# google-research/multinerf

Hardware: NVIDIA H100
Metric: train-step rays/sec @16384 rays x (64+64+32) samples (higher is better)
Workload: dtype bf16

## Files before the change

include/mnrf.h:

```cpp
#ifndef MNRF_H_
#define MNRF_H_

#include <stddef.h>
#include <stdint.h>

#ifdef __cplusplus
extern "C" {
#endif

typedef uint16_t mnrf_bf16;
typedef void* mnrf_stream;

#define MNRF_ABI_VERSION 2

int mnrf_abi_version(void);
const char* mnrf_last_error(void);
int mnrf_device_ok(void);
int mnrf_num_sms(void);

typedef struct {
  int32_t num_rays, num_prev, num_samples;
  int32_t use_dilation;
  float dilation, domain_lo, domain_hi;
  float anneal, resample_padding;
// ... 74 lines not shown
enum { MNRF_CHAIN_FWD = 0, MNRF_CHAIN_BWD = 1 };

typedef struct {
  const mnrf_bf16* w;
  int64_t ldw;
  const float* bias;
  uint32_t* maskbits;
  int64_t ldmaskbits;
  float* colsum;
  mnrf_bf16* out;
  int64_t ldo;
  int32_t n_stream, stream_col0, stream_kb0;
  int32_t n_res, res_kb0;
  int32_t reserved;
} mnrf_chain_layer;

typedef struct {
  int32_t mode, num_layers;
  int32_t width;
  int32_t stream_cols;
  int64_t m;
  const mnrf_bf16* stream;
  int64_t ldstream;
  const float* head_w;
  const float* head_b;
  float* head_out;
  int32_t head_n;
  int32_t reserved;
  mnrf_chain_layer layer[MNRF_CHAIN_MAX_LAYERS];
} mnrf_chain_desc;

int mnrf_mlp_chain(const mnrf_chain_desc* d, mnrf_stream stream);
int mnrf_mlp_chain_max_layers(void);

int mnrf_head_fwd(int64_t m, int32_t k, int32_t n_out, const mnrf_bf16* x, int64_t ldx,
                  const mnrf_bf16* w, const float* b, float* raw, mnrf_stream stream);
int mnrf_head_bwd(int64_t m, int32_t k, int32_t n_out, const mnrf_bf16* x, int64_t ldx,
                  const mnrf_bf16* w, const float* draw, mnrf_bf16* dx, int64_t lddx,
                  int32_t act, const mnrf_bf16* z, int64_t ldz, float* dw, float* dw2, int32_t dw_split,
                  float* db, float* dxsum, int32_t dx_cols, mnrf_bf16* dx2, int64_t lddx2, mnrf_stream stream);

enum { MNRF_HEAD_NONE = 0, MNRF_HEAD_FWD_SUB = 1, MNRF_HEAD_FWD_WARP = 2, MNRF_HEAD_BWD_SUB = 3,
       MNRF_HEAD_BWD_WARP = 4 };
typedef struct {
  int32_t fwd_kernel;
  int32_t fwd_lpr;
  int32_t fwd_grid;
  int32_t bwd_kernel;
  int32_t bwd_n_out;
  int32_t bwd_lpr;
  int32_t bwd_chunks;
  int32_t bwd_smooth;
  int32_t bwd_grid;
  int32_t reserved;
  int64_t fwd_rows_per_pass;
  int64_t bwd_rows_per_block;
} mnrf_head_instance;
int mnrf_head_plan(int64_t m, int32_t k, int32_t n_out, const mnrf_bf16* x, const mnrf_bf16* w, int32_t act,
                   const mnrf_bf16* z, const mnrf_bf16* dx, mnrf_head_instance* plan);

int mnrf_colsum(int64_t m, int32_t n, const mnrf_bf16* x, int64_t ldx, float* out,
                mnrf_stream stream);

enum { MNRF_RGB_SIGMOID = 0, MNRF_RGB_SAFE_EXP = 1 };

typedef struct {
// ... 218 lines not shown
```

multinerf_b200/csrc/chain.cu:

```cuda
#include <stdlib.h>
#include <string.h>

#include <algorithm>

#include "tc_common.cuh"

namespace mnrf {

constexpr int CH_W = 256;
constexpr int CH_ROWS = 128;
constexpr int CH_KBLK = CH_ROWS * 128;
constexpr int CH_WBLK = CH_W * 128;
constexpr int CH_RING = 4;
constexpr int CH_SEG = CH_W / 64;
constexpr int CH_SBLK = 64 * 128;
constexpr int CH_SRING = 3;
constexpr int CH_ACT = 4 * CH_KBLK;
constexpr int CH_THREADS = 384;
constexpr int CH_MAX_LAYERS = MNRF_CHAIN_MAX_LAYERS;
constexpr int CH_AUX = CH_MAX_LAYERS * CH_W * 4;
constexpr int CH_SMEM = CH_ACT + CH_RING * CH_WBLK + CH_SRING * CH_SBLK + CH_AUX + 256  + 1024 ;
static_assert(CH_SMEM <= 232448, "shared memory budget");
static_assert(CH_SEG >= 1 && CH_SEG <= CH_RING, "a segment must fit in the weight ring");

struct alignas(64) ChainMaps {
  CUtensorMap stream;
  CUtensorMap w[CH_MAX_LAYERS];
  CUtensorMap out[CH_MAX_LAYERS];
};

struct ChainLayer {
  int n_stream, stream_col0, stream_kb0;
  int n_res, res_kb0;
  int store;
  const float* bias;
  uint32_t* maskbits;
  int64_t ldmaskbits;
  float* colsum;
};

struct ChainParams {
  int num_layers;
  int64_t m;
  int64_t num_units;
  ChainLayer layer[CH_MAX_LAYERS];
  const float* head_w;
  const float* head_b;
  float* head_out;
};

__device__ __forceinline__ uint32_t pack_bf16_relu(float lo, float hi) {
  uint32_t r;
  asm("cvt.rn.relu.bf16x2.f32 %0, %1, %2;" : "=r"(r) : "f"(hi), "f"(lo));
  return r;
}

__device__ __forceinline__ float2 ld_shared_const_f2(uint32_t addr) {
  float2 v;
  asm("ld.shared.v2.f32 {%0, %1}, [%2];" : "=f"(v.x), "=f"(v.y) : "r"(addr));
  return v;
}

enum { CK_TURN, CK_FULL, CK_MMA, CK_EPI_SYNC, CK_EPI_LOOP, CK_EPI_TAIL, CK_N };
#ifdef MNRF_CHAIN_CLOCKS
__device__ unsigned long long g_chain_clk[CK_N];
#define CH_CLK(k) do { const long long t_ = clock64(); clk[k] += t_ - clk_t; clk_t = t_; } while (0)
#else
#define CH_CLK(k) do { } while (0)
#endif

template <int MODE, int NH>
__global__ void __launch_bounds__(CH_THREADS, 1)
mlp_chain_kernel(const __grid_constant__ ChainMaps maps, const ChainParams p) {
  extern __shared__ uint8_t smem_dyn[];
  uint8_t* smem = reinterpret_cast<uint8_t*>((reinterpret_cast<uintptr_t>(smem_dyn) + 1023) & ~uintptr_t(1023));
  uint8_t* act = smem;
  uint8_t* wring = act + CH_ACT;
  uint8_t* sring = wring + CH_RING * CH_WBLK;
  float* aux = reinterpret_cast<float*>(sring + CH_SRING * CH_SBLK);
  uint64_t* wfull = reinterpret_cast<uint64_t*>(aux + CH_MAX_LAYERS * CH_W);
  uint64_t* wempty = wfull + CH_RING;
  uint64_t* sfull = wempty + CH_RING;
  uint64_t* sempty = sfull + CH_SRING;
  uint64_t* turn = sempty + CH_SRING;

  const int warp = threadIdx.x >> 5;
  const int lane = threadIdx.x & 31;
  const int wg = threadIdx.x >> 7;

  if (threadIdx.x == 0) {
    bool any_stream = false;
    for (int j = 0; j < p.num_layers; ++j) {
      prefetch_tmap(&maps.w[j]);
      if (p.layer[j].store) prefetch_tmap(&maps.out[j]);
      any_stream |= p.layer[j].n_stream > 0;
    }
    if (any_stream) prefetch_tmap(&maps.stream);
    for (int i = 0; i < CH_RING; ++i) { mbar_init(&wfull[i], 1); mbar_init(&wempty[i], 8); }
    for (int i = 0; i < CH_SRING; ++i) { mbar_init(&sfull[i], 1); mbar_init(&sempty[i], 4); }
    for (int i = 0; i < 2; ++i) mbar_init(&turn[i], 4);
    fence_barrier_init();
  }
  if (MODE == 1)
    for (int i = threadIdx.x; i < CH_MAX_LAYERS * CH_W; i += CH_THREADS) aux[i] = 0.f;
  __syncthreads();
  pdl_launch_dependents();
  pdl_wait();
  if (MODE == 0) {
    for (int i = threadIdx.x; i < p.num_layers * CH_W; i += CH_THREADS) aux[i] = __ldg(p.layer[i / CH_W].bias + i % CH_W);
    __syncthreads();
  }

  if (wg == 0) {
    setmaxnreg_dec<40>();
    if (threadIdx.x == 0) {
      uint32_t wslot = 0, wphase = 0, sslot = 0, sphase = 0;
      for (int64_t unit = blockIdx.x; unit < p.num_units; unit += gridDim.x) {
        const int row0 = (int)(unit * CH_ROWS);
        for (int j = 0; j < p.num_layers; ++j) {
          const ChainLayer& L = p.layer[j];
          const int nk = L.n_res + L.n_stream;
          for (int s0 = 0; s0 < nk; s0 += CH_SEG) {
            const int s1 = min(s0 + CH_SEG, nk);
            for (int c = 0; c < 2; ++c)
              for (int s = s0; s < s1; ++s) {
                const bool streamed = s >= L.n_res;
                const int si = s - L.n_res;
                if (c == 0) {
                  mbar_wait(&wempty[wslot], wphase ^ 1, 1);
                  mbar_expect_tx(&wfull[wslot], CH_WBLK);
                  tma_load_2d(wring + wslot * CH_WBLK, &maps.w[j], &wfull[wslot],
                              (streamed ? L.stream_kb0 + si : L.res_kb0 + s) * 64, 0);
                  if (++wslot == CH_RING) { wslot = 0; wphase ^= 1; }
                }
                if (streamed) {
                  mbar_wait(&sempty[sslot], sphase ^ 1, 2);
                  mbar_expect_tx(&sfull[sslot], CH_SBLK);
                  tma_load_2d(sring + sslot * CH_SBLK, &maps.stream, &sfull[sslot], L.stream_col0 + si * 64, row0 + 64 * c);
                  if (++sslot == CH_SRING) { sslot = 0; sphase ^= 1; }
                }
              }
          }
          if (j == 0 && L.n_stream > 0 && unit + gridDim.x < p.num_units)
            for (int si = 0; si < L.n_stream; ++si)
              for (int c = 0; c < 2; ++c)
                tma_prefetch_2d(&maps.stream, L.stream_col0 + si * 64, (int)((unit + gridDim.x) * CH_ROWS) + 64 * c);
        }
      }
    }
  } else {
    setmaxnreg_inc<232>();
    const int c = wg - 1;
    const int w = warp & 3;
    const int r_in = 64 * c + 16 * w + (lane >> 2);
    const int q = lane & 3;
    const int cq = 2 * q;
    const uint32_t wring_s = smem_u32(wring), sring_s = smem_u32(sring), act_s = smem_u32(act);
    const uint32_t aux_s = smem_u32(aux);
    const bool lead = (threadIdx.x & 127) == 0;
    uint32_t wslot = 0, wphase = 0;
    uint32_t spos = 0;
    uint32_t seg = 0;
#ifdef MNRF_CHAIN_CLOCKS
    long long clk[CK_N] = {};
    long long clk_t = clock64();
#endif
    float acc[CH_W / 2];
    for (int64_t unit = blockIdx.x; unit < p.num_units; unit += gridDim.x) {
      int64_t rows[2];
      bool row_ok[2];
#pragma unroll
      for (int h = 0; h < 2; ++h) {
        rows[h] = unit * CH_ROWS + r_in + 8 * h;
        row_ok[h] = rows[h] < p.m;
      }
      for (int j = 0; j < p.num_layers; ++j) {
        const ChainLayer& L = p.layer[j];
        const bool last = (j == p.num_layers - 1);
        const bool do_head = (MODE == 0) && last && p.head_w != nullptr;
        uint32_t mw[2][2] = {{0u, 0u}, {0u, 0u}};
        if (MODE == 1 && L.maskbits) {
#pragma unroll
          for (int h = 0; h < 2; ++h)
#pragma unroll
            for (int e = 0; e < 2; ++e)
              if (row_ok[h]) mw[h][e] = __ldg(L.maskbits + rows[h] * L.ldmaskbits + 2 * q + e);
        }
        const int nk = L.n_res + L.n_stream;
        fence_acc(acc);
        for (int s0 = 0; s0 < nk; s0 += CH_SEG, ++seg) {
          const int s1 = min(s0 + CH_SEG, nk);
          const int ns = s1 - max(s0, L.n_res);
          uint32_t sp = spos + (c && ns > 0 ? ns : 0);
          if (ns > 0) spos += 2 * ns;
          if (c == 1) mbar_wait(&turn[1], seg & 1, 7);
          else if (seg > 0) mbar_wait(&turn[0], (seg - 1) & 1, 7);
          CH_CLK(CK_TURN);
          int prev_w = -1, prev_s = -1;
          for (int s = s0; s < s1; ++s) {
            const bool streamed = s >= L.n_res;
            mbar_wait(&wfull[wslot], wphase, 3);
            uint32_t a0 = act_s + s * CH_KBLK + c * (64 * 128);
            int cur_s = -1;
            if (streamed) {
              cur_s = (int)(sp % CH_SRING);
              mbar_wait(&sfull[cur_s], (sp / CH_SRING) & 1, 4);
              a0 = sring_s + cur_s * CH_SBLK;
              ++sp;
            }
            CH_CLK(CK_FULL);
            const uint32_t b0 = wring_s + wslot * CH_WBLK;
            wgmma_fence();
#pragma unroll
            for (int k = 0; k < 64 / WGMMA_K; ++k)
              Wgmma<CH_W, 0, 0>::mma(acc, make_smem_desc(a0 + k * (WGMMA_K * 2), 0, 1024),
                                     make_smem_desc(b0 + k * (WGMMA_K * 2), 0, 1024), (s > 0 || k > 0) ? 1u : 0u);
            wgmma_commit();
            wgmma_wait<1>();
            if (lane == 0) {
              if (prev_w >= 0) mbar_arrive(&wempty[prev_w]);
              if (prev_s >= 0) mbar_arrive(&sempty[prev_s]);
            }
            prev_w = (int)wslot;
            prev_s = cur_s;
            if (++wslot == CH_RING) { wslot = 0; wphase ^= 1; }
          }
          __syncwarp();
          if (lane == 0) mbar_arrive(&turn[c ^ 1]);
          wgmma_wait<0>();
          if (lane == 0) {
            mbar_arrive(&wempty[prev_w]);
            if (prev_s >= 0) mbar_arrive(&sempty[prev_s]);
          }
          CH_CLK(CK_MMA);
        }
        fence_acc(acc);

        if (lead) tma_store_wait_read<0>();
        named_bar_sync(1 + c, 128);
        CH_CLK(CK_EPI_SYNC);
        uint32_t bits[2] = {0u, 0u};
        float hdot[NH][2];
#pragma unroll
        for (int o = 0; o < NH; ++o) hdot[o][0] = hdot[o][1] = 0.f;
#pragma unroll
        for (int i = 0; i < CH_W / 8; ++i) {
          const int col = 8 * i + cq;
          float v[2][2];
#pragma unroll
          for (int h = 0; h < 2; ++h) { v[h][0] = acc[4 * i + 2 * h]; v[h][1] = acc[4 * i + 2 * h + 1]; }
          uint32_t o[2];
          if (MODE == 0) {
            const float2 b = ld_shared_const_f2(aux_s + (j * CH_W + col) * 4);
#pragma unroll
            for (int h = 0; h < 2; ++h) {
              v[h][0] += b.x;
              v[h][1] += b.y;
              bits[h] |= ((v[h][0] > 0.f ? 1u : 0u) | (v[h][1] > 0.f ? 2u : 0u)) << (col & 31);
              o[h] = pack_bf16_relu(v[h][0], v[h][1]);
            }
            if (do_head) {
#pragma unroll
              for (int oo = 0; oo < NH; ++oo) {
                const float2 hw = __ldg(reinterpret_cast<const float2*>(p.head_w + oo * CH_W + col));
#pragma unroll
                for (int h = 0; h < 2; ++h) hdot[oo][h] += bf16_lo(o[h]) * hw.x + bf16_hi(o[h]) * hw.y;
              }
            }
          } else {
            if (L.maskbits && (i & 3) == 0) {
#pragma unroll
              for (int h = 0; h < 2; ++h)
                bits[h] = __shfl_sync(0xffffffffu, mw[h][(i >> 2) & 1], (lane & ~3) | (i >> 3));
            }
#pragma unroll
            for (int h = 0; h < 2; ++h) {
              if (L.maskbits) {
                if (!((bits[h] >> (col & 31)) & 1u)) v[h][0] = 0.f;
                if (!((bits[h] >> ((col + 1) & 31)) & 1u)) v[h][1] = 0.f;
              }
              o[h] = pack_bf16(v[h][0], v[h][1]);
            }
            if (L.colsum) {
              float s0 = v[0][0] + v[1][0], s1 = v[0][1] + v[1][1];
#pragma unroll
              for (int sh = 4; sh < 32; sh <<= 1) {
                s0 += __shfl_xor_sync(0xffffffffu, s0, sh);
                s1 += __shfl_xor_sync(0xffffffffu, s1, sh);
              }
              if (lane < 4) { atomicAdd(aux + j * CH_W + col, s0); atomicAdd(aux + j * CH_W + col + 1, s1); }
            }
          }
#pragma unroll
          for (int h = 0; h < 2; ++h) {
            const int r = r_in + 8 * h;
            st_shared_u32(act_s + (col >> 6) * CH_KBLK + r * 128 + ((((col & 63) >> 3) ^ (r & 7)) << 4) + (cq << 1), o[h]);
          }
          if (MODE == 0 && (i & 3) == 3) {
#pragma unroll
            for (int h = 0; h < 2; ++h) {
              bits[h] |= __shfl_xor_sync(0xffffffffu, bits[h], 1);
              bits[h] |= __shfl_xor_sync(0xffffffffu, bits[h], 2);
              if (q == (i >> 3)) mw[h][(i >> 2) & 1] = bits[h];
              bits[h] = 0u;
            }
          }
        }
        CH_CLK(CK_EPI_LOOP);
        fence_proxy_async();
        named_bar_sync(1 + c, 128);
        CH_CLK(CK_EPI_SYNC);
        if (lead && L.store) {
#pragma unroll
          for (int kb = 0; kb < 4; ++kb)
            tma_store_2d(&maps.out[j], act + kb * CH_KBLK + c * (64 * 128), kb * 64, (int)(unit * CH_ROWS) + 64 * c);
          tma_store_commit();
        }
        if (MODE == 0 && L.maskbits) {
          const bool wide = (((uintptr_t)L.maskbits | (uintptr_t)(L.ldmaskbits * 4)) & 7) == 0;
#pragma unroll
          for (int h = 0; h < 2; ++h) {
            if (!row_ok[h]) continue;
            uint32_t* dst = L.maskbits + rows[h] * L.ldmaskbits + 2 * q;
            if (wide) *reinterpret_cast<uint2*>(dst) = make_uint2(mw[h][0], mw[h][1]);
            else { dst[0] = mw[h][0]; dst[1] = mw[h][1]; }
          }
        }
        if (do_head) {
#pragma unroll
          for (int oo = 0; oo < NH; ++oo)
#pragma unroll
            for (int h = 0; h < 2; ++h) {
              hdot[oo][h] += __shfl_xor_sync(0xffffffffu, hdot[oo][h], 1);
              hdot[oo][h] += __shfl_xor_sync(0xffffffffu, hdot[oo][h], 2);
              if (q == 0 && row_ok[h])
                p.head_out[rows[h] * NH + oo] = hdot[oo][h] + (p.head_b ? __ldg(p.head_b + oo) : 0.f);
            }
        }
        CH_CLK(CK_EPI_TAIL);
      }
    }
    if (lead) tma_store_wait_all();
#ifdef MNRF_CHAIN_CLOCKS
    if (blockIdx.x == 0 && threadIdx.x == 256)
      for (int k = 0; k < CK_N; ++k) atomicAdd(&g_chain_clk[k], (unsigned long long)clk[k]);
#endif
    if (MODE == 1) {
      named_bar_sync(3, 256);
      for (int jj = 0; jj < p.num_layers; ++jj) {
        if (!p.layer[jj].colsum) continue;
        for (int i = threadIdx.x - 128; i < CH_W; i += 256) atomicAdd(p.layer[jj].colsum + i, aux[jj * CH_W + i]);
      }
    }
  }
}

}

extern "C" int mnrf_mlp_chain_max_layers(void) { return mnrf::CH_MAX_LAYERS; }

#ifdef MNRF_CHAIN_CLOCKS
extern "C" int mnrf_chain_clocks(unsigned long long* out) {
  unsigned long long zero[mnrf::CK_N] = {};
  if (cudaDeviceSynchronize() != cudaSuccess) return 1;
  if (cudaMemcpyFromSymbol(out, mnrf::g_chain_clk, sizeof(zero)) != cudaSuccess) return 1;
  return cudaMemcpyToSymbol(mnrf::g_chain_clk, zero, sizeof(zero)) != cudaSuccess;
}
#endif

extern "C" int mnrf_mlp_chain(const mnrf_chain_desc* d, mnrf_stream stream_) {
  using namespace mnrf;
  cudaStream_t stream = (cudaStream_t)stream_;
  MNRF_CHECK(d, "mnrf_mlp_chain: null descriptor");
  MNRF_CHECK(d->m >= 0 && (d->m + CH_ROWS - 1) / CH_ROWS * CH_ROWS <= INT32_MAX,
             "mnrf_mlp_chain: m must be in [0, %d], got %lld", INT32_MAX / CH_ROWS * CH_ROWS, (long long)d->m);
  if (d->m == 0) return 0;
  MNRF_CHECK(d->mode == MNRF_CHAIN_FWD || d->mode == MNRF_CHAIN_BWD, "mnrf_mlp_chain: bad mode %d", d->mode);
  MNRF_CHECK(d->num_layers >= 1 && d->num_layers <= CH_MAX_LAYERS, "mnrf_mlp_chain: 1..%d layers, got %d",
             CH_MAX_LAYERS, d->num_layers);
  MNRF_CHECK(d->width == CH_W, "mnrf_mlp_chain: layer width must be %d, got %d", CH_W, d->width);
  const int sms = mnrf_num_sms();
  ChainMaps maps;
  memset(&maps, 0, sizeof(maps));
  ChainParams p{};
  p.num_layers = d->num_layers;
  p.m = d->m;
  p.num_units = (d->m + CH_ROWS - 1) / CH_ROWS;
  bool any_stream = false;
  for (int j = 0; j < d->num_layers; ++j) {
    const mnrf_chain_layer& s = d->layer[j];
    ChainLayer& L = p.layer[j];
    MNRF_CHECK(s.n_res == 0 || s.n_res == CH_W / 64, "mnrf_mlp_chain: layer %d: n_res must be 0 or %d", j, CH_W / 64);
    MNRF_CHECK(s.n_stream >= 0 && (s.n_stream > 0 || s.n_res > 0), "mnrf_mlp_chain: layer %d has no operand", j);
    MNRF_CHECK(s.stream_col0 >= 0 && s.stream_kb0 >= 0 && s.res_kb0 >= 0,
               "mnrf_mlp_chain: layer %d: negative column or k-block offset", j);
    MNRF_CHECK(j > 0 || s.n_res == 0, "mnrf_mlp_chain: the first layer has no resident operand");
    MNRF_CHECK(s.w && ((uintptr_t)s.w % 16) == 0 && s.ldw % 8 == 0, "mnrf_mlp_chain: layer %d: weights must be 16-byte aligned", j);
    const int kblocks = std::max(s.n_stream > 0 ? s.stream_kb0 + s.n_stream : 0, s.n_res > 0 ? s.res_kb0 + s.n_res : 0);
    MNRF_CHECK(s.ldw >= (int64_t)kblocks * 64, "mnrf_mlp_chain: layer %d: weight pitch %lld < K %d", j, (long long)s.ldw, kblocks * 64);
    L.n_stream = s.n_stream; L.stream_col0 = s.stream_col0; L.stream_kb0 = s.stream_kb0;
    L.n_res = s.n_res; L.res_kb0 = s.res_kb0;
    L.store = s.out ? 1 : 0;
    L.bias = s.bias; L.maskbits = s.maskbits; L.ldmaskbits = s.ldmaskbits; L.colsum = s.colsum;
    if (s.bias) MNRF_CHECK(((uintptr_t)s.bias % 8) == 0, "mnrf_mlp_chain: layer %d: bias must be 8-byte aligned", j);
    if (s.maskbits)
      MNRF_CHECK(s.ldmaskbits >= CH_W / 32, "mnrf_mlp_chain: layer %d: maskbits rows must hold >= %d words", j, CH_W / 32);
    if (d->mode == MNRF_CHAIN_BWD) MNRF_CHECK(!s.bias, "mnrf_mlp_chain: bias is a forward input");
    else MNRF_CHECK(s.bias && !s.colsum, "mnrf_mlp_chain: layer %d: the forward chain takes a bias and no colsum", j);
    if (make_tmap(&maps.w[j], s.w, CH_W, (int64_t)kblocks * 64, s.ldw, 64, CH_W)) return 1;
    if (s.out) {
      MNRF_CHECK(((uintptr_t)s.out % 16) == 0 && s.ldo % 8 == 0 && s.ldo >= CH_W, "mnrf_mlp_chain: layer %d: output alignment", j);
      if (make_tmap(&maps.out[j], s.out, d->m, CH_W, s.ldo, 64, 64)) return 1;
    }
    any_stream |= s.n_stream > 0;
    if (s.n_stream > 0)
      MNRF_CHECK(s.stream_col0 % 64 == 0 && s.stream_col0 + s.n_stream * 64 <= d->stream_cols,
                 "mnrf_mlp_chain: layer %d: streamed columns [%d, %d) outside the stream tensor (%d columns)", j,
                 s.stream_col0, s.stream_col0 + s.n_stream * 64, d->stream_cols);
  }
  if (any_stream) {
    MNRF_CHECK(d->stream && ((uintptr_t)d->stream % 16) == 0 && d->ldstream % 8 == 0 && d->stream_cols % 64 == 0,
               "mnrf_mlp_chain: streamed operand must be 16-byte aligned with a multiple of 64 columns");
    MNRF_CHECK(d->ldstream >= d->stream_cols, "mnrf_mlp_chain: stream pitch %lld < %d columns",
               (long long)d->ldstream, d->stream_cols);
    if (make_tmap(&maps.stream, d->stream, d->m, d->stream_cols, d->ldstream, 64, CH_ROWS / 2)) return 1;
  }
  p.head_w = d->head_w; p.head_b = d->head_b; p.head_out = d->head_out;
  const int head_n = d->head_n ? d->head_n : 1;
  if (d->head_w) MNRF_CHECK(d->mode == MNRF_CHAIN_FWD && d->head_out && ((uintptr_t)d->head_w % 16) == 0,
                            "mnrf_mlp_chain: the head is a forward output (16-byte aligned weights)");
  MNRF_CHECK(head_n == 1 || (head_n == 4 && d->head_w), "mnrf_mlp_chain: head_n must be 1 or 4, got %d", head_n);
  const int grid = (int)std::min<int64_t>(p.num_units, sms);
  const int rc = d->mode == MNRF_CHAIN_BWD ? launch_tc<mlp_chain_kernel<1, 1>>(grid, CH_THREADS, CH_SMEM, stream, maps, p)
                 : head_n == 4             ? launch_tc<mlp_chain_kernel<0, 4>>(grid, CH_THREADS, CH_SMEM, stream, maps, p)
                                           : launch_tc<mlp_chain_kernel<0, 1>>(grid, CH_THREADS, CH_SMEM, stream, maps, p);
  if (rc) return rc;
  MNRF_LAUNCH_CHECK();
  return 0;
}
```

multinerf_b200/lib.py:

```python
import ctypes as C
import os

import torch

_HERE = os.path.dirname(os.path.abspath(__file__))
LIB_PATH = os.environ.get('MNRF_LIB') or os.path.join(_HERE, 'libmnrf_b200.so')


class MnrfError(RuntimeError):
  pass


class SampleDesc(C.Structure):
  _fields_ = [('num_rays', C.c_int32), ('num_prev', C.c_int32), ('num_samples', C.c_int32),
              ('use_dilation', C.c_int32), ('dilation', C.c_float), ('domain_lo', C.c_float),
              ('domain_hi', C.c_float), ('anneal', C.c_float), ('resample_padding', C.c_float),
              ('jitter_mode', C.c_int32), ('max_jitter', C.c_float)]


class EncodeDesc(C.Structure):
  _fields_ = [('num_rays', C.c_int32), ('num_samples', C.c_int32), ('raydist_fn', C.c_int32),
              ('ray_shape', C.c_int32), ('warp_contract', C.c_int32),
              ('disable_integration', C.c_int32), ('basis_k', C.c_int32), ('min_deg', C.c_int32),
              ('max_deg', C.c_int32), ('ld_feat', C.c_int32), ('feat_cols', C.c_int32)]
# ... 52 lines not shown
class CameraDesc(C.Structure):
  _fields_ = [('num_rays', C.c_int32), ('num_cameras', C.c_int32), ('camtype', C.c_int32),
              ('has_distortion', C.c_int32), ('k1', C.c_float), ('k2', C.c_float), ('k3', C.c_float),
              ('k4', C.c_float), ('p1', C.c_float), ('p2', C.c_float), ('undistort_eps', C.c_float),
              ('undistort_iters', C.c_int32), ('has_ndc', C.c_int32), ('ndc_p02', C.c_float),
              ('ndc_p12', C.c_float), ('ndc_near', C.c_float)]


class SphericalDesc(C.Structure):
  _fields_ = [('height', C.c_int32), ('width', C.c_int32), ('camtoworld', C.c_double * 12)]


class PackItem(C.Structure):
  _fields_ = [('master', C.c_void_p), ('w_nk', C.c_void_p), ('w_kn', C.c_void_p), ('in_pad', C.c_int32),
              ('out', C.c_int32), ('tile0', C.c_int32), ('reserved', C.c_int32)]


CHAIN_MAX_LAYERS = 8
CHAIN_FWD, CHAIN_BWD = 0, 1


class ChainLayer(C.Structure):
  _fields_ = [('w', C.c_void_p), ('ldw', C.c_int64), ('bias', C.c_void_p), ('maskbits', C.c_void_p),
              ('ldmaskbits', C.c_int64), ('colsum', C.c_void_p), ('out', C.c_void_p), ('ldo', C.c_int64),
              ('n_stream', C.c_int32), ('stream_col0', C.c_int32), ('stream_kb0', C.c_int32),
              ('n_res', C.c_int32), ('res_kb0', C.c_int32), ('reserved', C.c_int32)]


class ChainDesc(C.Structure):
  _fields_ = [('mode', C.c_int32), ('num_layers', C.c_int32), ('width', C.c_int32), ('stream_cols', C.c_int32),
              ('m', C.c_int64), ('stream', C.c_void_p), ('ldstream', C.c_int64), ('head_w', C.c_void_p),
              ('head_b', C.c_void_p), ('head_out', C.c_void_p), ('head_n', C.c_int32), ('reserved', C.c_int32),
              ('layer', ChainLayer * CHAIN_MAX_LAYERS)]


class AdamDesc(C.Structure):
  _fields_ = [('n', C.c_int64), ('grad_max_val', C.c_float), ('grad_max_norm', C.c_float),
              ('lr', C.c_float), ('beta1', C.c_float), ('beta2', C.c_float), ('eps', C.c_float),
              ('step', C.c_int32), ('grad_scale', C.c_float)]


RAYDIST = {None: 0, 'none': 0, 'reciprocal': 1, 'log': 2, 'exp': 3, 'sqrt': 4, 'square': 5,
           'piecewise': 6}
RAY_SHAPE = {'cone': 0, 'cylinder': 1}
RGB_ACT = {'sigmoid': 0, 'safe_exp': 1}
LOSS_TYPE = {'mse': 0, 'charb': 1, 'rawnerf': 2}
GEMM_FWD, GEMM_DGRAD, GEMM_WGRAD = 0, 1, 2
ACT_NONE, ACT_RELU, ACT_SOFTPLUS, ACT_SILU = 0, 1, 2, 3
SMOOTH_ACTS = (ACT_SOFTPLUS, ACT_SILU)

_P = C.c_void_p
_SIGNATURES = {
    'mnrf_abi_version': (C.c_int, []),
    'mnrf_last_error': (C.c_char_p, []),
    'mnrf_device_ok': (C.c_int, []),
    'mnrf_num_sms': (C.c_int, []),
    'mnrf_sample_level': (C.c_int, [C.POINTER(SampleDesc)] + [_P] * 12),
    'mnrf_encode': (C.c_int, [C.POINTER(EncodeDesc)] + [_P] * 11 + [C.c_int32, _P]),
    'mnrf_viewdir_enc': (C.c_int, [C.c_int32, C.c_int32, C.c_int32, _P, _P, C.c_int32, C.c_int32,
                                   C.c_int32, _P]),
    'mnrf_gemm': (C.c_int, [C.POINTER(GemmDesc)] + [_P] * 10 + [C.c_int64, _P, _P]),
    'mnrf_gemm_wgrad': (C.c_int, [C.POINTER(GemmDesc)] + [_P] * 7),
    'mnrf_gemm_plan': (C.c_int, [C.POINTER(GemmDesc)] + [_P] * 10 + [C.c_int64] + [_P] * 4 +
                       [C.POINTER(GemmInstance)]),
    'mnrf_mlp_chain': (C.c_int, [C.POINTER(ChainDesc), _P]),
    'mnrf_mlp_chain_max_layers': (C.c_int, []),
    'mnrf_head_fwd': (C.c_int, [C.c_int64, C.c_int32, C.c_int32, _P, C.c_int64, _P, _P, _P, _P]),
    'mnrf_head_bwd': (C.c_int, [C.c_int64, C.c_int32, C.c_int32, _P, C.c_int64, _P, _P, _P, C.c_int64, C.c_int32,
                                _P, C.c_int64, _P, _P, C.c_int32, _P, _P, C.c_int32, _P, C.c_int64, _P]),
    'mnrf_head_plan': (C.c_int, [C.c_int64, C.c_int32, C.c_int32, _P, _P, C.c_int32, _P, _P, _P]),
    'mnrf_colsum': (C.c_int, [C.c_int64, C.c_int32, _P, C.c_int64, _P, _P]),
    'mnrf_composite_fwd': (C.c_int, [C.POINTER(CompositeDesc)] + [_P] * 18),
    'mnrf_composite_bwd': (C.c_int, [C.POINTER(LossDesc)] + [_P] * 24 + [C.c_int32, _P]),
    'mnrf_robust_mask': (C.c_int, [C.POINTER(RobustDesc)] + [_P] * 7 + [C.c_int32, _P]),
    'mnrf_quantile': (C.c_int, [C.c_int32, C.c_float, _P, _P, _P]),
    'mnrf_refdir_fwd': (C.c_int, [C.POINTER(RefdirDesc)] + [_P] * 10 + [C.c_float, C.c_float, C.c_int32, _P, _P]),
    'mnrf_refdir_bwd': (C.c_int, [C.POINTER(RefdirDesc)] + [_P] * 8 + [C.c_int32, C.c_float, C.c_float, C.c_int32] +
                        [_P] * 8),
    'mnrf_normals_fwd': (C.c_int, [C.c_int64, C.c_int32] + [_P] * 5 + [C.c_float, C.c_float, C.c_int32, _P, _P]),
    'mnrf_normals_bwd': (C.c_int, [C.c_int64, C.c_int32] + [_P] * 4 + [C.c_float, C.c_float, C.c_int32] + [_P] * 2 +
                         [C.c_int64] + [_P] * 3 +
                         [C.c_int64, _P, _P]),
    'mnrf_outer_mask': (C.c_int,[C.c_int64, C.c_int32, C.c_int64, _P, _P, _P, C.c_int64, _P, C.c_int64, _P]),
    'mnrf_act_tangent_bwd': (C.c_int, [C.c_int64, C.c_int32, C.c_int32] + [_P, C.c_int64] * 5 + [C.c_int32, _P]),
    'mnrf_pixels_to_rays': (C.c_int, [C.POINTER(CameraDesc)] + [_P] * 11),
    'mnrf_spherical_rays': (C.c_int, [C.POINTER(SphericalDesc)] + [_P] * 6),
    'mnrf_clip_adam': (C.c_int, [C.POINTER(AdamDesc)] + [_P] * 7),
    'mnrf_pack_weights_batched': (C.c_int, [C.c_int32, _P, C.c_int32, _P]),
    'mnrf_encode_points': (C.c_int, [C.POINTER(EncodeDesc), _P, C.c_float, _P, _P, _P, _P]),
    'mnrf_marching_cubes': (C.c_int, [C.c_int32] * 4 + [_P, C.c_float] + [_P] * 7),
    'mnrf_encode_points_tangent': (C.c_int, [C.POINTER(EncodeDesc), _P, C.c_float, _P, _P, _P, C.c_int32, _P]),
    'mnrf_point_rgb': (C.c_int, [C.POINTER(CompositeDesc), C.c_int64, _P, C.c_int32, _P, _P, _P, _P]),
    'mnrf_mc_normals': (C.c_int, [C.c_int32] * 3 + [_P, C.c_float] + [_P] * 4),
    'mnrf_tsdf_integrate': (C.c_int, [C.POINTER(CameraDesc)] + [C.c_int32] * 3 + [C.c_double] * 4 + [C.c_int32] * 3 +
                            [_P] * 5 + [C.c_float] + [_P] * 5),
    'mnrf_tsdf_integrate_contracted': (C.c_int, [C.POINTER(CameraDesc)] + [C.c_int32] * 3 + [C.c_double] * 4 +
                                       [C.c_int32] * 3 + [_P] * 5 + [C.c_float] + [_P] * 5),
    'mnrf_mesh_uncontract': (C.c_int, [C.c_int64] + [_P] * 5),
    'mnrf_mesh_components': (C.c_int, [C.c_int32, C.c_int64, _P, _P, _P]),
# ... 65 lines not shown
```

multinerf_b200/ops.py:

```python
import ctypes as C
import math
from typing import NamedTuple

import torch

from . import lib as L

EPS = float(torch.finfo(torch.float32).eps)

LAUNCHES = 0
GEMM_EVENTS = None


def _count(n=1):
  global LAUNCHES
  LAUNCHES += n


def _gemm_call(flops, fn, *args):
  _count()
  if GEMM_EVENTS is None:
    L.check(fn(*args))
    return
  ev = (torch.cuda.Event(enable_timing=True), torch.cuda.Event(enable_timing=True))
# ... 453 lines not shown
def chain_desc(mode, m, layers, *, stream=None, stream_cols=0, head_w=None, head_b=None, head_out=None, head_n=1):
  d = L.ChainDesc()
  d.mode, d.num_layers, d.width, d.stream_cols, d.m = mode, len(layers), 256, stream_cols, m
  if stream is not None:
    assert stream.dtype == torch.bfloat16 and stream.stride(1) == 1
    d.stream, d.ldstream = stream.data_ptr(), stream.stride(0)
  if head_w is not None:
    assert head_w.is_contiguous() and head_w.numel() == head_n * 256 and head_out.is_contiguous()
    d.head_w, d.head_out, d.head_n = head_w.data_ptr(), head_out.data_ptr(), head_n
    d.head_b = head_b.data_ptr() if head_b is not None else None
  flops = 0.0
  for j, ly in enumerate(layers):
    c = d.layer[j]
    w = ly['w']
    assert w.dtype == torch.bfloat16 and w.stride(1) == 1
    c.w, c.ldw = w.data_ptr(), w.stride(0)
    for name in ('bias', 'colsum'):
      t = ly.get(name)
      setattr(c, name, t.data_ptr() if t is not None else None)
    mb = ly.get('maskbits')
    if mb is not None:
      assert mb.dtype == torch.int32 and mb.stride(1) == 1
      c.maskbits, c.ldmaskbits = mb.data_ptr(), mb.stride(0)
    out = ly.get('out')
    if out is not None:
      assert out.dtype == torch.bfloat16 and out.stride(1) == 1
      c.out, c.ldo = out.data_ptr(), out.stride(0)
    c.n_stream, c.stream_col0, c.stream_kb0 = ly.get('n_stream', 0), ly.get('stream_col0', 0), ly.get('stream_kb0', 0)
    c.n_res, c.res_kb0 = ly.get('n_res', 0), ly.get('res_kb0', 0)
    flops += 2.0 * m * 256 * 64 * (c.n_stream + c.n_res)
  return d, flops


def mlp_chain(desc):
  lib = L.load()
  d, flops = desc
  _gemm_call(flops, lib.mnrf_mlp_chain, C.byref(d), L.stream_ptr())


def head_fwd(x, w_nk, bias, n_out, k, raw=None):
  lib = L.load()
  M = x.shape[0]
  if raw is None:
    raw = torch.empty(M, n_out, device=x.device)
  _count()
  L.check(lib.mnrf_head_fwd(M, k, n_out, L.ptr(x), x.stride(0), L.ptr(w_nk), L.ptr(bias),
                            L.ptr(raw), L.stream_ptr()))
  return raw


def head_bwd(x, w_nk, draw, n_out, k, dx=None, relu_mask=False, dw=None, db=None, dxsum=None, dw2=None, dw_split=0,
             dx_cols=0, dx2=None, act=L.ACT_NONE, z=None):
  lib = L.load()
  M = x.shape[0]
  if z is not None:
    assert not relu_mask and z.dtype == torch.bfloat16 and z.stride(-1) == 1
  else:
    act = L.ACT_RELU if relu_mask else L.ACT_NONE
  _count()
  L.check(lib.mnrf_head_bwd(M, k, n_out, L.ptr(x), x.stride(0), L.ptr(w_nk), L.ptr(_f32(draw)),
                            L.ptr(dx), dx.stride(0) if dx is not None else 0, act,
                            L.ptr(z), z.stride(0) if z is not None else 0, L.ptr(dw), L.ptr(dw2), int(dw_split),
                            L.ptr(db), L.ptr(dxsum), int(dx_cols), L.ptr(dx2), dx2.stride(0) if dx2 is not None else 0,
                            L.stream_ptr()))


# ... 234 lines not shown
```

Baseline: 289,700.

## Specialize MLP chain kernel into fixed forms for train, render and backward

Adds a FORM template parameter to the fused MLP chain kernel. A host-side classifier picks a specialized instantiation when all layers have masks and outputs (forward train, backward) or none have masks (render). The specialized forms fix mask and colsum branches at compile time, stage head weights in shared memory, and in backward read mask words from shared memory instead of warp shuffles. Forward mask packing is also changed to shift and pack the bits differently. The price is more template instantiations and a new planning API, and the bit-packing rewrite could break if its layout assumptions are off.

```diff
diff --git a/include/mnrf.h b/include/mnrf.h
--- a/include/mnrf.h
+++ b/include/mnrf.h
@@ -130,6 +130,17 @@
 
 int mnrf_mlp_chain(const mnrf_chain_desc* d, mnrf_stream stream);
 int mnrf_mlp_chain_max_layers(void);
+
+enum { MNRF_CHAIN_GENERIC = 0, MNRF_CHAIN_F_TRAIN = 1, MNRF_CHAIN_F_RENDER = 2, MNRF_CHAIN_B_MODEL = 3 };
+
+typedef struct {
+  int32_t form;
+  int32_t head_n;
+  int32_t smem_bytes;
+  int32_t reserved;
+} mnrf_chain_instance;
+
+int mnrf_chain_plan(const mnrf_chain_desc* d, mnrf_chain_instance* plan);
 
 int mnrf_head_fwd(int64_t m, int32_t k, int32_t n_out, const mnrf_bf16* x, int64_t ldx,
                   const mnrf_bf16* w, const float* b, float* raw, mnrf_stream stream);
diff --git a/multinerf_b200/csrc/chain.cu b/multinerf_b200/csrc/chain.cu
--- a/multinerf_b200/csrc/chain.cu
+++ b/multinerf_b200/csrc/chain.cu
@@ -19,9 +19,14 @@
 constexpr int CH_THREADS = 384;
 constexpr int CH_MAX_LAYERS = MNRF_CHAIN_MAX_LAYERS;
 constexpr int CH_AUX = CH_MAX_LAYERS * CH_W * 4;
-constexpr int CH_SMEM = CH_ACT + CH_RING * CH_WBLK + CH_SRING * CH_SBLK + CH_AUX + 256  + 1024 ;
+constexpr int CH_HEAD = CH_W * 4;
+constexpr int CH_SMEM = CH_ACT + CH_RING * CH_WBLK + CH_SRING * CH_SBLK + CH_AUX + CH_HEAD + 256  +
+                        1024 ;
 static_assert(CH_SMEM <= 232448, "shared memory budget");
 static_assert(CH_SEG >= 1 && CH_SEG <= CH_RING, "a segment must fit in the weight ring");
+
+enum { CH_GENERIC = MNRF_CHAIN_GENERIC, CH_F_TRAIN = MNRF_CHAIN_F_TRAIN, CH_F_RENDER = MNRF_CHAIN_F_RENDER,
+       CH_B_MODEL = MNRF_CHAIN_B_MODEL };
 
 struct alignas(64) ChainMaps {
   CUtensorMap stream;
@@ -69,16 +74,23 @@
 #define CH_CLK(k) do { } while (0)
 #endif
 
-template <int MODE, int NH>
+template <int MODE, int NH, int FORM>
 __global__ void __launch_bounds__(CH_THREADS, 1)
 mlp_chain_kernel(const __grid_constant__ ChainMaps maps, const ChainParams p) {
+  static_assert(FORM == CH_GENERIC || (FORM == CH_B_MODEL) == (MODE == 1), "a fixed form belongs to one mode");
+  static_assert(FORM == CH_GENERIC || NH == 1, "the fixed forward forms have one head output");
+  constexpr bool FIXED_FWD = FORM == CH_F_TRAIN || FORM == CH_F_RENDER;
+  constexpr bool MASKS_ALWAYS = FORM == CH_F_TRAIN || FORM == CH_B_MODEL;
+  constexpr bool MASKS_NEVER = FORM == CH_F_RENDER;
+  constexpr bool COLSUMS = MODE == 1 && FORM == CH_GENERIC;
   extern __shared__ uint8_t smem_dyn[];
   uint8_t* smem = reinterpret_cast<uint8_t*>((reinterpret_cast<uintptr_t>(smem_dyn) + 1023) & ~uintptr_t(1023));
   uint8_t* act = smem;
   uint8_t* wring = act + CH_ACT;
   uint8_t* sring = wring + CH_RING * CH_WBLK;
   float* aux = reinterpret_cast<float*>(sring + CH_SRING * CH_SBLK);
-  uint64_t* wfull = reinterpret_cast<uint64_t*>(aux + CH_MAX_LAYERS * CH_W);
+  float* headw = aux + CH_MAX_LAYERS * CH_W;
+  uint64_t* wfull = reinterpret_cast<uint64_t*>(headw + CH_W);
   uint64_t* wempty = wfull + CH_RING;
   uint64_t* sfull = wempty + CH_RING;
   uint64_t* sempty = sfull + CH_SRING;
@@ -101,13 +113,15 @@
     for (int i = 0; i < 2; ++i) mbar_init(&turn[i], 4);
     fence_barrier_init();
   }
-  if (MODE == 1)
+  if (COLSUMS)
     for (int i = threadIdx.x; i < CH_MAX_LAYERS * CH_W; i += CH_THREADS) aux[i] = 0.f;
   __syncthreads();
   pdl_launch_dependents();
   pdl_wait();
   if (MODE == 0) {
     for (int i = threadIdx.x; i < p.num_layers * CH_W; i += CH_THREADS) aux[i] = __ldg(p.layer[i / CH_W].bias + i % CH_W);
+    if (FIXED_FWD && p.head_w)
+      for (int i = threadIdx.x; i < CH_W; i += CH_THREADS) headw[i] = __ldg(p.head_w + i);
     __syncthreads();
   }
 
@@ -156,7 +170,7 @@
     const int q = lane & 3;
     const int cq = 2 * q;
     const uint32_t wring_s = smem_u32(wring), sring_s = smem_u32(sring), act_s = smem_u32(act);
-    const uint32_t aux_s = smem_u32(aux);
+    const uint32_t aux_s = smem_u32(aux), headw_s = smem_u32(headw);
     const bool lead = (threadIdx.x & 127) == 0;
     uint32_t wslot = 0, wphase = 0;
     uint32_t spos = 0;
@@ -178,8 +192,10 @@
         const ChainLayer& L = p.layer[j];
         const bool last = (j == p.num_layers - 1);
         const bool do_head = (MODE == 0) && last && p.head_w != nullptr;
+        const bool masks = MASKS_ALWAYS || (!MASKS_NEVER && L.maskbits != nullptr);
+        const bool colsum = COLSUMS && L.colsum != nullptr;
         uint32_t mw[2][2] = {{0u, 0u}, {0u, 0u}};
-        if (MODE == 1 && L.maskbits) {
+        if (MODE == 1 && masks) {
 #pragma unroll
           for (int h = 0; h < 2; ++h)
 #pragma unroll
@@ -240,6 +256,13 @@
         named_bar_sync(1 + c, 128);
         CH_CLK(CK_EPI_SYNC);
         uint32_t bits[2] = {0u, 0u};
+        uint32_t* mrow = reinterpret_cast<uint32_t*>(aux);
+        if (FORM == CH_B_MODEL) {
+#pragma unroll
+          for (int h = 0; h < 2; ++h)
+            *reinterpret_cast<uint2*>(mrow + (r_in + 8 * h) * 8 + 2 * q) = make_uint2(mw[h][0], mw[h][1]);
+          __syncwarp();
+        }
         float hdot[NH][2];
 #pragma unroll
         for (int o = 0; o < NH; ++o) hdot[o][0] = hdot[o][1] = 0.f;
@@ -256,32 +279,37 @@
             for (int h = 0; h < 2; ++h) {
               v[h][0] += b.x;
               v[h][1] += b.y;
-              bits[h] |= ((v[h][0] > 0.f ? 1u : 0u) | (v[h][1] > 0.f ? 2u : 0u)) << (col & 31);
+              if (!MASKS_NEVER)
+                bits[h] |= (v[h][0] > 0.f ? 1u << (8 * (i & 3)) : 0u) | (v[h][1] > 0.f ? 2u << (8 * (i & 3)) : 0u);
               o[h] = pack_bf16_relu(v[h][0], v[h][1]);
             }
             if (do_head) {
 #pragma unroll
               for (int oo = 0; oo < NH; ++oo) {
-                const float2 hw = __ldg(reinterpret_cast<const float2*>(p.head_w + oo * CH_W + col));
+                const float2 hw = FIXED_FWD ? ld_shared_const_f2(headw_s + col * 4)
+                                            : __ldg(reinterpret_cast<const float2*>(p.head_w + oo * CH_W + col));
 #pragma unroll
                 for (int h = 0; h < 2; ++h) hdot[oo][h] += bf16_lo(o[h]) * hw.x + bf16_hi(o[h]) * hw.y;
               }
             }
           } else {
-            if (L.maskbits && (i & 3) == 0) {
+            if (FORM == CH_B_MODEL && (i & 3) == 0) {
+#pragma unroll
+              for (int h = 0; h < 2; ++h) bits[h] = mrow[(r_in + 8 * h) * 8 + (i >> 2)];
+            } else if (masks && (i & 3) == 0) {
 #pragma unroll
               for (int h = 0; h < 2; ++h)
                 bits[h] = __shfl_sync(0xffffffffu, mw[h][(i >> 2) & 1], (lane & ~3) | (i >> 3));
             }
 #pragma unroll
             for (int h = 0; h < 2; ++h) {
-              if (L.maskbits) {
-                if (!((bits[h] >> (col & 31)) & 1u)) v[h][0] = 0.f;
-                if (!((bits[h] >> ((col + 1) & 31)) & 1u)) v[h][1] = 0.f;
+              if (masks) {
+                v[h][0] = (bits[h] >> (col & 31)) & 1u ? v[h][0] : 0.f;
+                v[h][1] = (bits[h] >> ((col + 1) & 31)) & 1u ? v[h][1] : 0.f;
               }
               o[h] = pack_bf16(v[h][0], v[h][1]);
             }
-            if (L.colsum) {
+            if (colsum) {
               float s0 = v[0][0] + v[1][0], s1 = v[0][1] + v[1][1];
 #pragma unroll
               for (int sh = 4; sh < 32; sh <<= 1) {
@@ -296,9 +324,10 @@
             const int r = r_in + 8 * h;
             st_shared_u32(act_s + (col >> 6) * CH_KBLK + r * 128 + ((((col & 63) >> 3) ^ (r & 7)) << 4) + (cq << 1), o[h]);
           }
-          if (MODE == 0 && (i & 3) == 3) {
+          if (MODE == 0 && !MASKS_NEVER && (i & 3) == 3) {
 #pragma unroll
             for (int h = 0; h < 2; ++h) {
+              bits[h] <<= cq;
               bits[h] |= __shfl_xor_sync(0xffffffffu, bits[h], 1);
               bits[h] |= __shfl_xor_sync(0xffffffffu, bits[h], 2);
               if (q == (i >> 3)) mw[h][(i >> 2) & 1] = bits[h];
@@ -316,8 +345,8 @@
             tma_store_2d(&maps.out[j], act + kb * CH_KBLK + c * (64 * 128), kb * 64, (int)(unit * CH_ROWS) + 64 * c);
           tma_store_commit();
         }
-        if (MODE == 0 && L.maskbits) {
-          const bool wide = (((uintptr_t)L.maskbits | (uintptr_t)(L.ldmaskbits * 4)) & 7) == 0;
+        if (MODE == 0 && masks) {
+          const bool wide = FORM == CH_F_TRAIN || (((uintptr_t)L.maskbits | (uintptr_t)(L.ldmaskbits * 4)) & 7) == 0;
 #pragma unroll
           for (int h = 0; h < 2; ++h) {
             if (!row_ok[h]) continue;
@@ -345,7 +374,7 @@
     if (blockIdx.x == 0 && threadIdx.x == 256)
       for (int k = 0; k < CK_N; ++k) atomicAdd(&g_chain_clk[k], (unsigned long long)clk[k]);
 #endif
-    if (MODE == 1) {
+    if (COLSUMS) {
       named_bar_sync(3, 256);
       for (int jj = 0; jj < p.num_layers; ++jj) {
         if (!p.layer[jj].colsum) continue;
@@ -368,9 +397,9 @@
 }
 #endif
 
-extern "C" int mnrf_mlp_chain(const mnrf_chain_desc* d, mnrf_stream stream_) {
-  using namespace mnrf;
-  cudaStream_t stream = (cudaStream_t)stream_;
+namespace mnrf {
+
+static int chain_check(const mnrf_chain_desc* d) {
   MNRF_CHECK(d, "mnrf_mlp_chain: null descriptor");
   MNRF_CHECK(d->m >= 0 && (d->m + CH_ROWS - 1) / CH_ROWS * CH_ROWS <= INT32_MAX,
              "mnrf_mlp_chain: m must be in [0, %d], got %lld", INT32_MAX / CH_ROWS * CH_ROWS, (long long)d->m);
@@ -379,6 +408,80 @@
   MNRF_CHECK(d->num_layers >= 1 && d->num_layers <= CH_MAX_LAYERS, "mnrf_mlp_chain: 1..%d layers, got %d",
              CH_MAX_LAYERS, d->num_layers);
   MNRF_CHECK(d->width == CH_W, "mnrf_mlp_chain: layer width must be %d, got %d", CH_W, d->width);
+  bool any_stream = false;
+  for (int j = 0; j < d->num_layers; ++j) {
+    const mnrf_chain_layer& s = d->layer[j];
+    MNRF_CHECK(s.n_res == 0 || s.n_res == CH_W / 64, "mnrf_mlp_chain: layer %d: n_res must be 0 or %d", j, CH_W / 64);
+    MNRF_CHECK(s.n_stream >= 0 && (s.n_stream > 0 || s.n_res > 0), "mnrf_mlp_chain: layer %d has no operand", j);
+    MNRF_CHECK(s.stream_col0 >= 0 && s.stream_kb0 >= 0 && s.res_kb0 >= 0,
+               "mnrf_mlp_chain: layer %d: negative column or k-block offset", j);
+    MNRF_CHECK(j > 0 || s.n_res == 0, "mnrf_mlp_chain: the first layer has no resident operand");
+    MNRF_CHECK(s.w && ((uintptr_t)s.w % 16) == 0 && s.ldw % 8 == 0, "mnrf_mlp_chain: layer %d: weights must be 16-byte aligned", j);
+    const int kblocks = std::max(s.n_stream > 0 ? s.stream_kb0 + s.n_stream : 0, s.n_res > 0 ? s.res_kb0 + s.n_res : 0);
+    MNRF_CHECK(s.ldw >= (int64_t)kblocks * 64, "mnrf_mlp_chain: layer %d: weight pitch %lld < K %d", j, (long long)s.ldw, kblocks * 64);
+    if (s.bias) MNRF_CHECK(((uintptr_t)s.bias % 8) == 0, "mnrf_mlp_chain: layer %d: bias must be 8-byte aligned", j);
+    if (s.maskbits)
+      MNRF_CHECK(s.ldmaskbits >= CH_W / 32, "mnrf_mlp_chain: layer %d: maskbits rows must hold >= %d words", j, CH_W / 32);
+    if (d->mode == MNRF_CHAIN_BWD) MNRF_CHECK(!s.bias, "mnrf_mlp_chain: bias is a forward input");
+    else MNRF_CHECK(s.bias && !s.colsum, "mnrf_mlp_chain: layer %d: the forward chain takes a bias and no colsum", j);
+    if (s.out)
+      MNRF_CHECK(((uintptr_t)s.out % 16) == 0 && s.ldo % 8 == 0 && s.ldo >= CH_W, "mnrf_mlp_chain: layer %d: output alignment", j);
+    any_stream |= s.n_stream > 0;
+    if (s.n_stream > 0)
+      MNRF_CHECK(s.stream_col0 % 64 == 0 && s.stream_col0 + s.n_stream * 64 <= d->stream_cols,
+                 "mnrf_mlp_chain: layer %d: streamed columns [%d, %d) outside the stream tensor (%d columns)", j,
+                 s.stream_col0, s.stream_col0 + s.n_stream * 64, d->stream_cols);
+  }
+  if (any_stream) {
+    MNRF_CHECK(d->stream && ((uintptr_t)d->stream % 16) == 0 && d->ldstream % 8 == 0 && d->stream_cols % 64 == 0,
+               "mnrf_mlp_chain: streamed operand must be 16-byte aligned with a multiple of 64 columns");
+    MNRF_CHECK(d->ldstream >= d->stream_cols, "mnrf_mlp_chain: stream pitch %lld < %d columns",
+               (long long)d->ldstream, d->stream_cols);
+  }
+  const int head_n = d->head_n ? d->head_n : 1;
+  if (d->head_w) MNRF_CHECK(d->mode == MNRF_CHAIN_FWD && d->head_out && ((uintptr_t)d->head_w % 16) == 0,
+                            "mnrf_mlp_chain: the head is a forward output (16-byte aligned weights)");
+  MNRF_CHECK(head_n == 1 || (head_n == 4 && d->head_w), "mnrf_mlp_chain: head_n must be 1 or 4, got %d", head_n);
+  return 0;
+}
+
+static int chain_form(const mnrf_chain_desc* d) {
+  const int nl = std::min(std::max(d->num_layers, 0), CH_MAX_LAYERS);
+  bool all_masks = true, no_masks = true, all_out = true, any_colsum = false, early_out = false, masks_wide = true;
+  for (int j = 0; j < nl; ++j) {
+    const mnrf_chain_layer& s = d->layer[j];
+    all_masks &= s.maskbits != nullptr;
+    no_masks &= s.maskbits == nullptr;
+    all_out &= s.out != nullptr;
+    any_colsum |= s.colsum != nullptr;
+    early_out |= j < nl - 1 && s.out != nullptr;
+    if (s.maskbits) masks_wide &= (((uintptr_t)s.maskbits | (uintptr_t)(s.ldmaskbits * 4)) & 7) == 0;
+  }
+  if (d->mode == MNRF_CHAIN_BWD) return all_masks && all_out && !any_colsum ? CH_B_MODEL : CH_GENERIC;
+  if (d->head_n == 4) return CH_GENERIC;
+  if (all_masks && all_out && masks_wide) return CH_F_TRAIN;
+  if (no_masks && !early_out) return CH_F_RENDER;
+  return CH_GENERIC;
+}
+
+}
+
+extern "C" int mnrf_chain_plan(const mnrf_chain_desc* d, mnrf_chain_instance* plan) {
+  using namespace mnrf;
+  MNRF_CHECK(plan, "mnrf_chain_plan: null plan");
+  if (chain_check(d)) return 1;
+  memset(plan, 0, sizeof(*plan));
+  plan->form = chain_form(d);
+  plan->head_n = d->head_n ? d->head_n : 1;
+  plan->smem_bytes = CH_SMEM;
+  return 0;
+}
+
+extern "C" int mnrf_mlp_chain(const mnrf_chain_desc* d, mnrf_stream stream_) {
+  using namespace mnrf;
+  cudaStream_t stream = (cudaStream_t)stream_;
+  if (chain_check(d)) return 1;
+  if (d->m == 0) return 0;
   const int sms = mnrf_num_sms();
   ChainMaps maps;
   memset(&maps, 0, sizeof(maps));
@@ -390,50 +493,29 @@
   for (int j = 0; j < d->num_layers; ++j) {
     const mnrf_chain_layer& s = d->layer[j];
     ChainLayer& L = p.layer[j];
-    MNRF_CHECK(s.n_res == 0 || s.n_res == CH_W / 64, "mnrf_mlp_chain: layer %d: n_res must be 0 or %d", j, CH_W / 64);
-    MNRF_CHECK(s.n_stream >= 0 && (s.n_stream > 0 || s.n_res > 0), "mnrf_mlp_chain: layer %d has no operand", j);
-    MNRF_CHECK(s.stream_col0 >= 0 && s.stream_kb0 >= 0 && s.res_kb0 >= 0,
-               "mnrf_mlp_chain: layer %d: negative column or k-block offset", j);
-    MNRF_CHECK(j > 0 || s.n_res == 0, "mnrf_mlp_chain: the first layer has no resident operand");
-    MNRF_CHECK(s.w && ((uintptr_t)s.w % 16) == 0 && s.ldw % 8 == 0, "mnrf_mlp_chain: layer %d: weights must be 16-byte aligned", j);
     const int kblocks = std::max(s.n_stream > 0 ? s.stream_kb0 + s.n_stream : 0, s.n_res > 0 ? s.res_kb0 + s.n_res : 0);
-    MNRF_CHECK(s.ldw >= (int64_t)kblocks * 64, "mnrf_mlp_chain: layer %d: weight pitch %lld < K %d", j, (long long)s.ldw, kblocks * 64);
     L.n_stream = s.n_stream; L.stream_col0 = s.stream_col0; L.stream_kb0 = s.stream_kb0;
     L.n_res = s.n_res; L.res_kb0 = s.res_kb0;
     L.store = s.out ? 1 : 0;
     L.bias = s.bias; L.maskbits = s.maskbits; L.ldmaskbits = s.ldmaskbits; L.colsum = s.colsum;
-    if (s.bias) MNRF_CHECK(((uintptr_t)s.bias % 8) == 0, "mnrf_mlp_chain: layer %d: bias must be 8-byte aligned", j);
-    if (s.maskbits)
-      MNRF_CHECK(s.ldmaskbits >= CH_W / 32, "mnrf_mlp_chain: layer %d: maskbits rows must hold >= %d words", j, CH_W / 32);
-    if (d->mode == MNRF_CHAIN_BWD) MNRF_CHECK(!s.bias, "mnrf_mlp_chain: bias is a forward input");
-    else MNRF_CHECK(s.bias && !s.colsum, "mnrf_mlp_chain: layer %d: the forward chain takes a bias and no colsum", j);
     if (make_tmap(&maps.w[j], s.w, CH_W, (int64_t)kblocks * 64, s.ldw, 64, CH_W)) return 1;
-    if (s.out) {
-      MNRF_CHECK(((uintptr_t)s.out % 16) == 0 && s.ldo % 8 == 0 && s.ldo >= CH_W, "mnrf_mlp_chain: layer %d: output alignment", j);
-      if (make_tmap(&maps.out[j], s.out, d->m, CH_W, s.ldo, 64, 64)) return 1;
-    }
+    if (s.out && make_tmap(&maps.out[j], s.out, d->m, CH_W, s.ldo, 64, 64)) return 1;
     any_stream |= s.n_stream > 0;
-    if (s.n_stream > 0)
-      MNRF_CHECK(s.stream_col0 % 64 == 0 && s.stream_col0 + s.n_stream * 64 <= d->stream_cols,
-                 "mnrf_mlp_chain: layer %d: streamed columns [%d, %d) outside the stream tensor (%d columns)", j,
-                 s.stream_col0, s.stream_col0 + s.n_stream * 64, d->stream_cols);
-  }
-  if (any_stream) {
-    MNRF_CHECK(d->stream && ((uintptr_t)d->stream % 16) == 0 && d->ldstream % 8 == 0 && d->stream_cols % 64 == 0,
-               "mnrf_mlp_chain: streamed operand must be 16-byte aligned with a multiple of 64 columns");
-    MNRF_CHECK(d->ldstream >= d->stream_cols, "mnrf_mlp_chain: stream pitch %lld < %d columns",
-               (long long)d->ldstream, d->stream_cols);
-    if (make_tmap(&maps.stream, d->stream, d->m, d->stream_cols, d->ldstream, 64, CH_ROWS / 2)) return 1;
-  }
+  }
+  if (any_stream && make_tmap(&maps.stream, d->stream, d->m, d->stream_cols, d->ldstream, 64, CH_ROWS / 2)) return 1;
   p.head_w = d->head_w; p.head_b = d->head_b; p.head_out = d->head_out;
   const int head_n = d->head_n ? d->head_n : 1;
-  if (d->head_w) MNRF_CHECK(d->mode == MNRF_CHAIN_FWD && d->head_out && ((uintptr_t)d->head_w % 16) == 0,
-                            "mnrf_mlp_chain: the head is a forward output (16-byte aligned weights)");
-  MNRF_CHECK(head_n == 1 || (head_n == 4 && d->head_w), "mnrf_mlp_chain: head_n must be 1 or 4, got %d", head_n);
   const int grid = (int)std::min<int64_t>(p.num_units, sms);
-  const int rc = d->mode == MNRF_CHAIN_BWD ? launch_tc<mlp_chain_kernel<1, 1>>(grid, CH_THREADS, CH_SMEM, stream, maps, p)
-                 : head_n == 4             ? launch_tc<mlp_chain_kernel<0, 4>>(grid, CH_THREADS, CH_SMEM, stream, maps, p)
-                                           : launch_tc<mlp_chain_kernel<0, 1>>(grid, CH_THREADS, CH_SMEM, stream, maps, p);
+  int rc;
+  switch (chain_form(d)) {
+    case CH_F_TRAIN: rc = launch_tc<mlp_chain_kernel<0, 1, CH_F_TRAIN>>(grid, CH_THREADS, CH_SMEM, stream, maps, p); break;
+    case CH_F_RENDER: rc = launch_tc<mlp_chain_kernel<0, 1, CH_F_RENDER>>(grid, CH_THREADS, CH_SMEM, stream, maps, p); break;
+    case CH_B_MODEL: rc = launch_tc<mlp_chain_kernel<1, 1, CH_B_MODEL>>(grid, CH_THREADS, CH_SMEM, stream, maps, p); break;
+    default:
+      rc = d->mode == MNRF_CHAIN_BWD ? launch_tc<mlp_chain_kernel<1, 1, CH_GENERIC>>(grid, CH_THREADS, CH_SMEM, stream, maps, p)
+           : head_n == 4 ? launch_tc<mlp_chain_kernel<0, 4, CH_GENERIC>>(grid, CH_THREADS, CH_SMEM, stream, maps, p)
+                         : launch_tc<mlp_chain_kernel<0, 1, CH_GENERIC>>(grid, CH_THREADS, CH_SMEM, stream, maps, p);
+  }
   if (rc) return rc;
   MNRF_LAUNCH_CHECK();
   return 0;
diff --git a/multinerf_b200/lib.py b/multinerf_b200/lib.py
--- a/multinerf_b200/lib.py
+++ b/multinerf_b200/lib.py
@@ -108,6 +108,15 @@
               ('m', C.c_int64), ('stream', C.c_void_p), ('ldstream', C.c_int64), ('head_w', C.c_void_p),
               ('head_b', C.c_void_p), ('head_out', C.c_void_p), ('head_n', C.c_int32), ('reserved', C.c_int32),
               ('layer', ChainLayer * CHAIN_MAX_LAYERS)]
+
+
+class ChainInstance(C.Structure):
+  _fields_ = [('form', C.c_int32), ('head_n', C.c_int32), ('smem_bytes', C.c_int32), ('reserved', C.c_int32)]
+
+
+CHAIN_GENERIC, CHAIN_F_TRAIN, CHAIN_F_RENDER, CHAIN_B_MODEL = 0, 1, 2, 3
+CHAIN_FORMS = {CHAIN_GENERIC: 'generic', CHAIN_F_TRAIN: 'F-train', CHAIN_F_RENDER: 'F-render',
+               CHAIN_B_MODEL: 'B-model'}
 
 
 class AdamDesc(C.Structure):
@@ -141,6 +150,7 @@
                        [C.POINTER(GemmInstance)]),
     'mnrf_mlp_chain': (C.c_int, [C.POINTER(ChainDesc), _P]),
     'mnrf_mlp_chain_max_layers': (C.c_int, []),
+    'mnrf_chain_plan': (C.c_int, [C.POINTER(ChainDesc), _P]),
     'mnrf_head_fwd': (C.c_int, [C.c_int64, C.c_int32, C.c_int32, _P, C.c_int64, _P, _P, _P, _P]),
     'mnrf_head_bwd': (C.c_int, [C.c_int64, C.c_int32, C.c_int32, _P, C.c_int64, _P, _P, _P, C.c_int64, C.c_int32,
                                 _P, C.c_int64, _P, _P, C.c_int32, _P, _P, C.c_int32, _P, C.c_int64, _P]),
diff --git a/multinerf_b200/ops.py b/multinerf_b200/ops.py
--- a/multinerf_b200/ops.py
+++ b/multinerf_b200/ops.py
@@ -509,6 +509,15 @@
   return d, flops
 
 
+def chain_plan(desc):
+  lib = L.load()
+  plan = L.ChainInstance()
+  L.check(lib.mnrf_chain_plan(C.byref(desc[0]), C.byref(plan)))
+  out = {name: int(getattr(plan, name)) for name, _ in L.ChainInstance._fields_ if name != 'reserved'}
+  out['form_name'] = L.CHAIN_FORMS[out['form']]
+  return out
+
+
 def mlp_chain(desc):
   lib = L.load()
   d, flops = desc
```

Result: faster. 294,000 (median of 6 runs) (+1.5%).
